# chalharu/rust-compression

Hardware: AMD Instinct MI355X
Metric: BZip2 level-9 encode MB/s (input bytes, HBM-resident in and out: the kernels' rate; value_end_to_end is host buffer to host buffer at the C ABI) (higher is better)
Workload: dtype u8/u32

## Files before the change

### rust-compression_amd/csrc/bzgpu.h

```cpp
#pragma once
#include <hip/hip_runtime.h>
#include <stdint.h>
#include <stddef.h>

namespace bzgpu {

typedef uint8_t u8;
typedef uint16_t u16;
typedef uint32_t u32;
typedef uint64_t u64;
typedef int64_t i64;

constexpr u32 kWave = 64;
constexpr u32 kMaxBlockLen = 900000;
constexpr u32 kSortTile = 8192;
constexpr u32 kSortThreads = 512;
constexpr u32 kTilesPerBlock = 110;
constexpr u32 kSlot = kTilesPerBlock * kSortTile;
constexpr u32 kPtSlot = kSlot / 8u * 10u;
constexpr u32 kPairWords = 65536u / 32u;
constexpr u32 kMaxBins = 2048;
constexpr u32 kPerK = 8;
constexpr u32 kGSize = 50;
constexpr u32 kMaxSelectors = 18002;
// ... 200 lines not shown
        if (nbytes & 1u) r = gf_mulmod(r, xp2[k]);
    return r;
}

__device__ __forceinline__ u32 crc_bytes_raw(const u8 *__restrict__ p, u64 len, const u32 *s_tab)
{
    u32 crc = 0;
    for (u64 i = 0; i < len; ++i) crc = s_tab[(crc >> 24) ^ p[i]] ^ (crc << 8);
    return crc;
}


struct RleBuffers {
    i64 *tile_last;
    i64 *carry_in;
    u32 *tile_crc;
    u32 *tile_count;
    u16 *sub_off;
    i64 *sub_rs;
    u64 *tile_off;
    u64 *total;
    u64 *cut_result;
    u64 *scan_part;
};

struct CutPlan {
    u64 L;
    u64 g_base;
    u64 own_hi;
    u64 w_min;
    u64 j_lo, j_hi;
    u64 tb, t1;
    u64 t_last;
    u64 t_eval;
};
struct CutBuffers {
    u64 *step_t0;
    u32 *step_nt;
    u64 *step_w0;
    u32 *tab;
    u16 *comp;
};

struct BwtArgs {
    const u8 *rle;
    const BlockDesc *blocks;
// ... 163 lines not shown
void launch_dec_crc(hipStream_t st, const DecArgs &a, const u64 *out_base, const u8 *out, u32 max_out_len,
                    const u32 *crc_tab, const u32 *xp2, const u32 *xp16);

enum KernelId {
    KID_RADIX_HIST = 0,
    KID_RADIX_SCAN,
    KID_RADIX_SCATTER,
    KID_GROUP_FLAGS,
    KID_GROUP_APPLY,
    KID_LAST_COLUMN,
    KID_RADIX_SCATTER_LB,
    KID_GHIST_TEXT,
    KID_GHIST_SCAN,
    KID_RANK_PLACE,
    KID_PHASE_B_LOCAL,
    KID_GROUP_REFINE,
    KID_DEC_BLOCK,
    KID_DEC_MTF,
    KID_DEC_TSORT,
    KID_DEC_WALK,
    KID_DEC_PLACE,
    KID_DEC_RLE,
    KID_DEC_CRC,
    KID_COUNT
};
struct KernelProf {
    bool on = false;
    struct Rec {
        int id;
        u64 bytes;
        hipEvent_t a, b;
    };
    Rec *recs = nullptr;
    u32 nrecs = 0, cap = 0;
    u64 launches[KID_COUNT] = {};
    u64 bytes[KID_COUNT] = {};
    double seconds[KID_COUNT] = {};
    int begin(hipStream_t st, int id, u64 nbytes);
    void end(hipStream_t st, int idx);
    void set_bytes(int idx, u64 nbytes) { if (idx >= 0) recs[idx].bytes = nbytes; }
    void collect();
    void reset();
};

void launch_slab_last(hipStream_t st, const RleBuffers &rb, u64 t0, u64 t1, i64 *d_out);
void launch_rle_scan(hipStream_t st, const u8 *d_in, u64 n, u64 t0, u64 t1, u64 in_begin, const u32 *crc_tab,
                     const u32 *xp16, const RleBuffers &rb);
void launch_rle_count(hipStream_t st, const u8 *d_in, u64 n, u64 t0, u64 t1, u64 in_begin, i64 init_carry,
                      const RleBuffers &rb, i64 *d_out_last);
void launch_rle_prefix(hipStream_t st, u64 tb, u64 t1, const RleBuffers &rb, bool write_end = true);
void launch_rle_cuts(hipStream_t st, const u8 *d_in, u64 n, u64 tb, u64 t1, u64 in_begin, const RleBuffers &rb,
                     u32 block_max_len, int emit_tail, BlockDesc *d_blocks, u32 max_blocks);
void launch_rle_image(hipStream_t st, const u8 *d_in, u64 n, u64 tb, u64 t1, u64 in_begin, const RleBuffers &rb, u8 *d_rle);
u64 cut_table_entries(const CutPlan &pl);
void cut_groups(const CutPlan &pl, u64 *g_lo, u64 *g_hi, u64 *entries);
u32 cut_seg_cap();
void launch_cut_steps(hipStream_t st, const CutPlan &pl, const RleBuffers &rb, const CutBuffers &cb);
void launch_cut_tables(hipStream_t st, const CutPlan &pl, const u8 *d_in, u64 n_lim, const RleBuffers &rb, const CutBuffers &cb,
                       u64 work_total);
void launch_cut_select(hipStream_t st, const CutPlan &pl, u64 j0, u64 s0, u64 start_in, u64 n, long long rle_bias, int emit_tail,
                       const RleBuffers &rb, const CutBuffers &cb, BlockDesc *d_blocks, u32 max_blocks);
void launch_block_crc(hipStream_t st, const u8 *d_in, const BlockDesc *d_blocks, u32 nblocks,
                      const u32 *crc_tab, const u32 *xp2, const u32 *tile_crc, u32 *d_crc);
void launch_block_symbols(hipStream_t st, const BwtArgs &a, u32 *inuse_bits, u8 *sym_code, u8 *keyinfo);
int run_bwt(hipStream_t st, const BwtArgs &a, u32 max_n, u64 total_n, unsigned long long *h_active,
            u64 *sorted_elems, KernelProf *prof, u64 *round_active , bool wide_keys,
            u32 min_chars);
void launch_mtf(hipStream_t st, const MtfArgs &a);
inline bool env_verify() { return getenv("BZ_VERIFY") && atoi(getenv("BZ_VERIFY")) != 0; }
struct MailSeg {
    void *h;
    const void *d;
    size_t n;
};
int mail_fetch(hipStream_t st, const MailSeg *segs, int nseg);
void mail_release(hipStream_t st);
// ... 12 lines not shown
```

### rust-compression_amd/csrc/engine.hip

```cpp
#include "engine_state.h"

#include <algorithm>
#include <chrono>
#include <cstdio>
#include <cstdlib>
#include <cstring>
#include <vector>

#define MAILCHK(st, ...)                                                             \
    do {                                                                             \
        const MailSeg mail_segs_[] = {__VA_ARGS__};                                  \
        if (mail_fetch((st), mail_segs_, (int)(sizeof(mail_segs_) / sizeof(mail_segs_[0]))) != 0) return BZ_E_UNEXPECTED; \
    } while (0)

static int span_begin(bz_gpu_engine *g, int stage, hipStream_t st = nullptr)
{
    bz_gpu_engine::Span s;
    s.stage = stage;
    s.st = st ? st : g->st;
    if (hipEventCreate(&s.a) != hipSuccess || hipEventCreate(&s.b) != hipSuccess) return -1;
    (void)hipEventRecord(s.a, s.st);
    g->spans.push_back(s);
    return (int)g->spans.size() - 1;
}
// ... 184 lines not shown
    df_workspace_free(g->df);
    if (g->h_active) (void)hipHostFree(g->h_active);
    mail_release(g->st);
    mail_release(g->st2);
    if (g->st) (void)hipStreamDestroy(g->st);
    if (g->ev_aux) (void)hipEventDestroy(g->ev_aux);
    if (g->st2) (void)hipStreamDestroy(g->st2);
    delete g;
}

static RleBuffers rle_buffers(bz_gpu_engine *g)
{
    RleBuffers rb;
    rb.tile_last = g->tile_last.as<i64>();
    rb.carry_in = g->carry_in.as<i64>();
    rb.tile_crc = g->tile_crc.as<u32>();
    rb.tile_count = g->tile_count.as<u32>();
    rb.tile_off = g->tile_off.as<u64>();
    rb.sub_off = g->sub_off.as<u16>();
    rb.sub_rs = g->sub_rs.as<i64>();
    rb.total = g->scal.as<u64>();
    rb.cut_result = g->scal.as<u64>() + 2;
    rb.scan_part = g->scan_part.as<u64>();
    return rb;
}

extern "C" int bz_gpu_partition_slab_begin(bz_gpu_engine *g, int level, const void *d_in, size_t n,
                                           uint64_t tile0, uint64_t tile1, int64_t *slab_last_start)
{
    if (!g || level < 1 || level > 9) return BZ_E_PARAM;
    if (n && ((uintptr_t)d_in & 15u)) return BZ_E_PARAM;
    HIPCHK(hipSetDevice(g->device));
    const u64 ntiles = (n + kRleTile - 1) / kRleTile;
    if (tile1 > ntiles) tile1 = ntiles;
    if (tile0 > tile1) tile0 = tile1;
    g->level = level;
    g->d_in = (const u8 *)d_in;
    g->n_in = n;
    g->slab_t0 = tile0;
    g->slab_t1 = tile1;
    g->h_blocks.clear();
    g->h_crc.clear();
    for (double &t : g->t_stage) t = 0;
    for (u64 &s : g->bwt_stats) s = 0;
    for (u64 &s : g->round_active) s = 0;
    if (slab_last_start) *slab_last_start = -1;
    if (ntiles == 0) return BZ_OK;
    int rc;
    if ((rc = g->tile_last.ensure(ntiles * 8)) || (rc = g->carry_in.ensure(ntiles * 8)) ||
        (rc = g->tile_crc.ensure(ntiles * 4)) || (rc = g->tile_count.ensure(ntiles * 4)) ||
        (rc = g->tile_off.ensure((ntiles + 1) * 8)) || (rc = g->sub_off.ensure(ntiles * 32)) ||
        (rc = g->sub_rs.ensure(ntiles * 128)) || (rc = g->scal.ensure(128)) ||
        (rc = g->scan_part.ensure((ntiles / 1024 + 2) * 8)))
        return rc;
    const RleBuffers rb = rle_buffers(g);
    const int sp = span_begin(g, 0);
    launch_rle_scan(g->st, g->d_in, n, tile0, tile1, 0, g->crc_tab.as<u32>(), g->xp16.as<u32>(), rb);
    i64 *d_last = reinterpret_cast<i64 *>(g->scal.as<u64>() + 8);
    if (tile1 > tile0) {
        launch_slab_last(g->st, rb, tile0, tile1, d_last);
        i64 last = -1;
        span_end(g, sp);
        MAILCHK(g->st, {&last, d_last, 8});
        if (slab_last_start) *slab_last_start = last;
    } else {
        span_end(g, sp);
    }
    HIPCHK(hipGetLastError());
    return BZ_OK;
}

extern "C" int bz_gpu_partition_slab_count(bz_gpu_engine *g, int64_t carry_run)
{
    if (!g) return BZ_E_PARAM;
    HIPCHK(hipSetDevice(g->device));
    if (g->slab_t1 <= g->slab_t0) return BZ_OK;
    const RleBuffers rb = rle_buffers(g);
    const int sp = span_begin(g, 0);
    const u64 ntiles = (g->n_in + kRleTile - 1) / kRleTile;
    launch_rle_count(g->st, g->d_in, g->n_in, g->slab_t0, g->slab_t1, 0, carry_run, rb,
                     g->slab_t1 < ntiles ? rb.carry_in + g->slab_t1 : nullptr);
    span_end(g, sp);
    HIPCHK(hipGetLastError());
    return BZ_OK;
}

struct SlabCuts {
    u64 tb = 0, start_in = 0;
    size_t nb = 0;
    int span = -1;
    bool pending = false, image_done = false;
};
static bool cut_tables_enabled()
{
    static const bool on = [] {
        const char *e = getenv("BZ_CUT_TABLES");
        return !(e && atoi(e) == 0);
    }();
    return on;
// ... 65 lines not shown
}

static int slab_cuts(bz_gpu_engine *g, uint64_t start_in, int is_last, bool image_beside, SlabCuts &sc, size_t *n_blocks,
                     uint64_t *next_in, int *tail_block)
{
    sc = SlabCuts();
    HIPCHK(hipSetDevice(g->device));
    if (n_blocks) *n_blocks = 0;
    if (next_in) *next_in = start_in;
    if (tail_block) *tail_block = 0;
    const u64 n = g->n_in;
    if (n == 0) return BZ_OK;
    const u64 t0 = g->slab_t0, t1 = g->slab_t1;
    u64 tb = start_in / kRleTile;
    if (tb > t0) tb = t0;
    if (start_in > t0 * (u64)kRleTile) return BZ_E_PARAM;
    const RleBuffers rb = rle_buffers(g);
    const u32 block_max_len = (u32)g->level * 100000u - 19u;
    sc.span = span_begin(g, 0);
    if (tb < t0) {
        launch_rle_scan(g->st, g->d_in, n, tb, t0, start_in, g->crc_tab.as<u32>(), g->xp16.as<u32>(), rb);
        launch_rle_count(g->st, g->d_in, n, tb, t0, start_in, -1, rb, nullptr);
    }
    launch_rle_prefix(g->st, tb, t1, rb);
    u64 total = 0;
    MAILCHK(g->st, {&total, rb.total, 8});
    const size_t max_blocks = (size_t)(total / block_max_len + 2);
    int rc;
    if ((rc = g->rle.ensure(total + 256)) || (rc = g->blocks_all.ensure(max_blocks * sizeof(BlockDesc))) ||
        (rc = g->crc_all.ensure(max_blocks * 4)))
        return rc;
    const bool tables = start_in == 0 && t0 == 0 && cut_tables_enabled();
    if (image_beside) {
        if (!g->ev_aux) HIPCHK(hipEventCreateWithFlags(&g->ev_aux, hipEventDisableTiming));
        if (tables) {
            launch_rle_image(g->st2, g->d_in, n, tb, t1, start_in, rb, g->rle.as<u8>());
            HIPCHK(hipEventRecord(g->ev_aux, g->st2));
            sc.image_done = true;
        }
    }
    u64 res[5] = {~0ull, 0, 0, 0, 0};
    if (tables) {
        if ((rc = cut_tables_prepare(g, 0, total, tb, t1)) != BZ_OK) return rc;
        if (g->cut_ready && (rc = cut_tables_select(g, 0, 0, 0, 0, is_last ? 1 : 0, (u32)max_blocks, res)) != BZ_OK) return rc;
        if (res[0] == ~0ull) {
            if (g->cut_ready) fprintf(stderr, "bz2_mi355x: the cut tables did not answer a target; the chain kernel takes over\n");
            ++g->cut_stats[1];
        } else {
            ++g->cut_stats[0];
        }
    }
    if (res[0] == ~0ull) {
        launch_rle_cuts(g->st, g->d_in, n, tb, t1, start_in, rb, block_max_len, is_last ? 1 : 0,
                        g->blocks_all.as<BlockDesc>(), (u32)max_blocks);
        if (image_beside && !sc.image_done) {
            launch_rle_image(g->st2, g->d_in, n, tb, t1, start_in, rb, g->rle.as<u8>());
            HIPCHK(hipEventRecord(g->ev_aux, g->st2));
            sc.image_done = true;
        }
        MAILCHK(g->st, {res, rb.cut_result, 3 * sizeof(u64)});
    }
    if (image_beside) HIPCHK(hipStreamWaitEvent(g->st, g->ev_aux, 0));
    const size_t nb = (size_t)res[0];
    if (nb > max_blocks) return BZ_E_UNEXPECTED;
    sc.tb = tb;
    sc.start_in = start_in;
    sc.nb = nb;
    sc.pending = true;
    if (n_blocks) *n_blocks = nb;
    if (next_in) *next_in = nb || is_last ? res[1] : start_in;
    if (tail_block) *tail_block = (int)res[2];
    return BZ_OK;
}
static int slab_image(bz_gpu_engine *g, SlabCuts &sc)
{
    if (!sc.pending) return BZ_OK;
    sc.pending = false;
    const RleBuffers rb = rle_buffers(g);
    if (!sc.image_done) launch_rle_image(g->st, g->d_in, g->n_in, sc.tb, g->slab_t1, sc.start_in, rb, g->rle.as<u8>());
    const size_t nb = sc.nb;
    g->h_blocks.resize(nb);
    g->h_crc.resize(nb);
    if (nb) {
        launch_block_crc(g->st, g->d_in, g->blocks_all.as<BlockDesc>(), (u32)nb, g->crc_tab.as<u32>(),
                         g->xp2.as<u32>(), g->tile_crc.as<u32>(), g->crc_all.as<u32>());
    }
    span_end(g, sc.span);
    if (nb) MAILCHK(g->st, {g->h_blocks.data(), g->blocks_all.p, nb * sizeof(BlockDesc)}, {g->h_crc.data(), g->crc_all.p, nb * 4});
    spans_collect(g);
    HIPCHK(hipGetLastError());
    return BZ_OK;
}

struct SlabSpec {
    u64 total = 0;
    u64 g_base = 0;
    u64 halo_cap = 0;
    bool image_done = false;
    u64 want_halo_total = 0;
};
static int slab_spec_total(bz_gpu_engine *g, SlabSpec &sp)
{
    sp = SlabSpec();
    if (g->n_in == 0) return BZ_OK;
    HIPCHK(hipSetDevice(g->device));
    const RleBuffers rb = rle_buffers(g);
    const int span = span_begin(g, 0);
    launch_rle_prefix(g->st, g->slab_t0, g->slab_t1, rb);
    span_end(g, span);
    MAILCHK(g->st, {&sp.total, rb.total, 8});
    return BZ_OK;
}
static int slab_spec_tables(bz_gpu_engine *g, SlabSpec &sp, u64 g_base)
{
    sp.g_base = g_base;
    g->cut_ready = false;
    if (g->n_in == 0) return BZ_OK;
    const u64 L = (u64)g->level * 100000u - 19u;
    sp.halo_cap = g_base ? (L + 8u + 255u) / 256u * 256u : 0u;
    const size_t max_blocks = (size_t)((sp.total + L + 4u) / L + 2u);
    int rc;
    if ((rc = g->rle.ensure(sp.halo_cap + sp.total + 256)) || (rc = g->blocks_all.ensure(max_blocks * sizeof(BlockDesc))) ||
        (rc = g->crc_all.ensure(max_blocks * 4)))
        return rc;
    const RleBuffers rb = rle_buffers(g);
    const int span = span_begin(g, 0);
    if (!g->ev_aux) HIPCHK(hipEventCreateWithFlags(&g->ev_aux, hipEventDisableTiming));
    launch_rle_image(g->st2, g->d_in, g->n_in, g->slab_t0, g->slab_t1, 0, rb, g->rle.as<u8>() + sp.halo_cap);
    HIPCHK(hipEventRecord(g->ev_aux, g->st2));
    sp.image_done = true;
    rc = cut_tables_prepare(g, g_base, sp.total, g->slab_t0, g->slab_t1);
    span_end(g, span);
    return rc;
}
static int slab_spec_select(bz_gpu_engine *g, SlabSpec &sp, u64 start_in, u64 s0, u64 j0, int is_last, SlabCuts &sc,
                            size_t *n_blocks, u64 *next_in, u64 *s_next, u64 *j_next)
{
    sc = SlabCuts();
    *n_blocks = 0;
    *next_in = start_in;
    *s_next = s0;
    *j_next = j0;
    if (g->n_in == 0) return BZ_OK;
    const u64 t0 = g->slab_t0;
    if (start_in > t0 * (u64)kRleTile || s0 > sp.g_base) return BZ_E_PARAM;
    const u64 L = (u64)g->level * 100000u - 19u;
    const u64 D = sp.g_base - s0;
    if (D > sp.halo_cap) return BZ_E_UNEXPECTED;
    const size_t max_blocks = (size_t)((sp.total + L + 4u) / L + 2u);
    u64 res[5] = {~0ull, 0, 0, 0, 0};
    int rc;
// ... 22 lines not shown
    sc.pending = true;
    sc.image_done = true;
    sc.span = -1;
    *n_blocks = sc.nb;
    *next_in = sc.nb || is_last ? res[1] : start_in;
    *s_next = res[3];
    *j_next = res[4];
    sp.want_halo_total = D;
    return BZ_OK;
}
static int slab_spec_finish(bz_gpu_engine *g, SlabSpec &sp, SlabCuts &sc)
{
    if (!sc.pending) return BZ_OK;
    if (!sp.image_done) return slab_image(g, sc);
    const RleBuffers rb = rle_buffers(g);
    const u64 t0 = g->slab_t0;
    sc.span = span_begin(g, 0);
    g->h_halo_total = sp.want_halo_total;
    if (sc.tb < t0) {
        launch_rle_scan(g->st, g->d_in, g->n_in, sc.tb, t0, sc.start_in, g->crc_tab.as<u32>(), g->xp16.as<u32>(), rb);
        launch_rle_count(g->st, g->d_in, g->n_in, sc.tb, t0, sc.start_in, -1, rb, nullptr);
        launch_rle_prefix(g->st, sc.tb, t0, rb, false);
        HIPCHK(hipMemcpyAsync(&g->h_halo_total, rb.total, 8, hipMemcpyDeviceToHost, g->st));
        launch_rle_image(g->st, g->d_in, g->n_in, sc.tb, t0, sc.start_in, rb, g->rle.as<u8>() + sp.halo_cap - sp.want_halo_total);
    }
    HIPCHK(hipStreamWaitEvent(g->st, g->ev_aux, 0));
    return slab_image(g, sc);
}

extern "C" int bz_gpu_partition_slab_finish(bz_gpu_engine *g, uint64_t start_in, int is_last, size_t *n_blocks,
                                            uint64_t *next_in, int *tail_block)
{
    if (!g) return BZ_E_PARAM;
    SlabCuts sc;
    const int rc = slab_cuts(g, start_in, is_last, true, sc, n_blocks, next_in, tail_block);
    if (rc != BZ_OK) {
        if (sc.span >= 0) { span_end(g, sc.span); spans_collect(g); }
        return rc;
    }
    return slab_image(g, sc);
}

extern "C" int bz_gpu_partition(bz_gpu_engine *g, int level, const void *d_in, size_t n, int mode,
                                size_t *n_blocks, size_t *consumed, int *tail_block)
{
    if (!g || level < 1 || level > 9) return BZ_E_PARAM;
    if (n_blocks) *n_blocks = 0;
// ... 931 lines not shown
        if (total >= (1u << 20)) return BZ_E_PARAM;
    }
    HIPCHK(hipSetDevice(g->device));
    DevBuf f, o, s, fl;
    int rc;
    if ((rc = f.ensure(alpha * 4)) || (rc = o.ensure(alpha + 8)) || (rc = s.ensure((size_t)kLmWords * 4)) ||
        (rc = fl.ensure(4)))
        return rc;
    HIPCHK(hipMemcpyAsync(f.p, h_freq, alpha * 4, hipMemcpyHostToDevice, g->st));
    launch_probe_code_lengths(g->st, f.as<u32>(), (u32)alpha, o.as<u8>(), s.as<u32>(), fl.as<int>());
    int flag = 0;
    HIPCHK(hipMemcpyAsync(h_len, o.p, alpha, hipMemcpyDeviceToHost, g->st));
    HIPCHK(hipMemcpyAsync(&flag, fl.p, 4, hipMemcpyDeviceToHost, g->st));
    HIPCHK(hipStreamSynchronize(g->st));
    HIPCHK(hipGetLastError());
    if (took_length_limited_path) *took_length_limited_path = flag;
    return BZ_OK;
}

static const char *kKernelNames[KID_COUNT] = {"k_radix_hist", "k_radix_scan", "k_radix_scatter",
                                              "k_group_flags", "k_group_apply", "k_last_column",
                                              "k_radix_scatter_lb", "k_ghist_text", "k_ghist_scan", "k_rank_place", "k_phase_b_local", "k_group_refine",
                                              "k_dec_block", "k_dec_mtf", "k_dec_tsort", "k_dec_walk_lengths",
                                              "k_dec_place", "k_dec_rle", "k_dec_crc"};

extern "C" int bz_gpu_profile_enable(bz_gpu_engine *g, int on)
{
    if (!g) return BZ_E_PARAM;
    g->prof.reset();
    g->prof.on = (on & 1) != 0;
    g->debug_figures = (on & 2) != 0;
    return BZ_OK;
}

extern "C" int bz_gpu_profile_kernels(bz_gpu_engine *g)
{
    (void)g;
    return KID_COUNT;
}

extern "C" int bz_gpu_profile_get(bz_gpu_engine *g, int idx, const char **name, uint64_t *launches,
                                  double *seconds, uint64_t *algorithmic_bytes)
{
    if (!g || idx < 0 || idx >= KID_COUNT) return BZ_E_PARAM;
    if (name) *name = kKernelNames[idx];
    if (launches) *launches = g->prof.launches[idx];
    if (seconds) *seconds = g->prof.seconds[idx];
// ... 4 lines not shown
```

### rust-compression_amd/csrc/engine_state.h

```cpp
#pragma once
#include "../../include/bz2_mi355x.h"
#include "bzgpu.h"
#include "dev_buf.h"

#include <cstdio>
#include <vector>

using namespace bzgpu;

struct DecWorkspace;
void dec_workspace_free(DecWorkspace *w);
int dec_decode_for_verify(struct bz_gpu_engine *g, const uint8_t *d_in, uint64_t n, uint8_t *d_out, uint64_t cap,
                          uint64_t *produced, int *verdict);
struct bz_gpu_engine *dec_cache_take(int device, int prefer = 0);
void dec_cache_put(int device, struct bz_gpu_engine *g);
void dec_release_cached();
struct DfWorkspace;
void df_workspace_free(DfWorkspace *w);

#define HIPCHK(x)                                                                                     \
    do {                                                                                              \
        hipError_t e_ = (x);                                                                          \
        if (e_ != hipSuccess) {                                                                       \
            fprintf(stderr, "bz2_mi355x: HIP error %s at %s:%d\n", hipGetErrorString(e_), __FILE__,   \
                    __LINE__);                                                                        \
            return BZ_E_UNEXPECTED;                                                                   \
        }                                                                                             \
    } while (0)

struct bz_gpu_engine {
    int device = 0;
    hipStream_t st = nullptr;
    hipStream_t st2 = nullptr;
    size_t max_blocks = 0;

    DevBuf crc_tab, xp16, xp2;
    DevBuf tile_last, carry_in, tile_crc, tile_count, tile_off, sub_off, sub_rs, scal, scan_part, rle, blocks_all, crc_all;
    DevBuf cut_step_t0, cut_step_nt, cut_step_w0, cut_tab, cut_comp;
    CutPlan cut_plan = {};
    bool cut_ready = false;
    u64 h_halo_total = 0;
    u64 cut_stats[2] = {0, 0};
    std::vector<BlockDesc> h_blocks;
    std::vector<u32> h_crc;
    const u8 *d_in = nullptr;
    u64 n_in = 0;
    u64 slab_t0 = 0, slab_t1 = 0;
    int level = 9;
    DevBuf lblocks, lcrc, SA, R, KA, VA, KB, VB, tile_hist, count, flags, tlo, tln, nonfinal, active, per_k,
        per_shift, lin_p, lin_sig, bin_cursor, pb_gate, bin_base, newbits, sym_code, keyinfo, count2, tile_nf, L, orig_ptr, inuse_bits, summ, summ_len, init_state, rank8, ptext, pair_bits, ztile_last, ztile_cnt, zstate, ztick, mtf,
        mtf_freq, bout, selector, code_len, group_bitoff, lm_scratch, hglen, hpack, hrfreq, hlm, hpass, stream, error_flag, packlist, gh_tiles, gbase,
        tile_state, tickets;
    u32 sort_epoch = 0;
    bool zle_fused_broken = false;
    u32 fused_state[2] = {0, 0};
    hipEvent_t ev_aux = nullptr;
    size_t ws_blocks = 0;
    DevBuf packed, gathered, asmlist;
    unsigned long long *h_active = nullptr;
    std::vector<BlockOut> h_out;
    std::vector<u32> h_out_nblock;
    std::vector<u32> h_out_pass;
    double t_stage[6] = {0, 0, 0, 0, 0, 0};
    KernelProf prof;
    double shard_ms[8] = {0, 0, 0, 0, 0, 0, 0, 0};
// ... 19 lines not shown
```

### rust-compression_amd/csrc/k_rle1.hip

```cpp
#include "bzgpu.h"

namespace bzgpu {

constexpr u32 RT = 256;

__device__ __forceinline__ i64 block_excl_max64(i64 v, i64 *sh , i64 &total)
{
    const u32 l = lane_id(), w = threadIdx.x >> 6;
    i64 inc = wave_incl_max64(v);
    if (l == 63) sh[w] = inc;
    __syncthreads();
    i64 carry = -1;
    for (u32 k = 0; k < w; ++k) carry = sh[k] > carry ? sh[k] : carry;
    i64 tot = -1;
    for (u32 k = 0; k < RT / 64; ++k) tot = sh[k] > tot ? sh[k] : tot;
    total = tot;
    i64 prev = __shfl_up(inc, 1, 64);
    i64 ex = (l == 0) ? (i64)-1 : prev;
    __syncthreads();
    return ex > carry ? ex : carry;
}

__device__ __forceinline__ u32 block_excl_sum(u32 v, u32 *sh , u32 &total)
{
// ... 300 lines not shown
    __shared__ __attribute__((aligned(16))) u8 s_out[2 * kRleTile + 32];
    const u64 tile = t0 + blockIdx.x;
    Seg s;
    load_seg(in, n, tile, s, in_begin);
    const i64 rs = seg_run_start(s, carry_in[tile], s_m);
    u8 e[16], cph[16];
    const u32 cnt = eval_seg(s, rs, e, cph);
    u32 tot;
    u8 *dst = rle + tile_off[tile];
    const u32 a0 = (u32)(reinterpret_cast<uintptr_t>(dst) & 15u);
    u32 o = a0 + block_excl_sum(cnt, s_s, tot);
#pragma unroll
    for (u32 k = 0; k < 16; ++k) {
        if (e[k]) {
            if (cph[k] < 4u) s_out[o++] = s.b[k];
            if (e[k] == 2u || cph[k] >= 4u) s_out[o++] = (u8)(cph[k] - 3u);
        }
    }
    __syncthreads();
    u8 *line0 = dst - a0;
    const u32 end = a0 + tot, nlines = (end + 15u) >> 4;
    for (u32 j = threadIdx.x; j < nlines; j += RT) {
        const u32 lo = j * 16u;
        if (lo >= a0 && lo + 16u <= end) {
            *reinterpret_cast<uint4 *>(line0 + lo) = *reinterpret_cast<const uint4 *>(s_out + lo);
        } else {
            const u32 b0 = lo > a0 ? lo : a0, b1 = lo + 16u < end ? lo + 16u : end;
            for (u32 b = b0; b < b1; ++b) line0[b] = s_out[b];
        }
    }
}

constexpr u32 CW = 16;
constexpr u32 CT = CW * 64;
constexpr u32 CSW_SMALL = 2, CSW_BIG = 12;
constexpr u32 CSEG = CSW_BIG * 64;
constexpr u64 CUT_END = ~0ull, CUT_OUT = ~0ull - 1;

__global__ __launch_bounds__(CT) void k_rle_cuts(const u8 *__restrict__ in, u64 n, u64 t_begin, u64 in_begin,
                                                  const u16 *__restrict__ sub_off,
                                                  const i64 *__restrict__ sub_rs,
                                                  const u64 *__restrict__ tile_off, u64 ntiles,
                                                  u32 block_max_len, int emit_tail,
                                                  BlockDesc *__restrict__ blocks, u32 max_blocks,
                                                  u64 *__restrict__ out_nblocks_consumed )
{
// ... 560 lines not shown
        if (write_end) (void)hipMemsetAsync(rb.tile_off + tb, 0, 8, st);
        return;
    }
    tiles_scan<false>(st, rb.tile_count, rb.tile_off, tb, t1, rb.scan_part, 0ull, rb.total, write_end ? rb.tile_off + t1 : nullptr);
}

void launch_rle_cuts(hipStream_t st, const u8 *d_in, u64 n, u64 tb, u64 t1, u64 in_begin, const RleBuffers &rb,
                     u32 block_max_len, int emit_tail, BlockDesc *d_blocks, u32 max_blocks)
{
    if (t1 <= tb) {
        (void)hipMemsetAsync(rb.cut_result, 0, 3 * sizeof(u64), st);
        return;
    }
    hipLaunchKernelGGL(k_rle_cuts, dim3(1), dim3(CT), 0, st, d_in, n, tb, in_begin, rb.sub_off, rb.sub_rs,
                       rb.tile_off, t1, block_max_len, emit_tail, d_blocks, max_blocks, rb.cut_result);
}
void launch_rle_image(hipStream_t st, const u8 *d_in, u64 n, u64 tb, u64 t1, u64 in_begin, const RleBuffers &rb, u8 *d_rle)
{
    if (t1 <= tb) return;
    hipLaunchKernelGGL(k_rle_scatter, dim3((u32)(t1 - tb)), dim3(RT), 0, st, d_in, n, tb, in_begin, rb.carry_in,
                       rb.tile_off, d_rle);
}

u64 cut_table_entries(const CutPlan &pl) { return pl.j_hi >= pl.j_lo ? cut_tbase(pl.j_lo, pl.j_hi + 1u) : 0u; }
void cut_groups(const CutPlan &pl, u64 *g_lo, u64 *g_hi, u64 *entries)
{
    *g_lo = (pl.j_lo + 15u) / 16u;
    *g_hi = *g_lo;
    *entries = 0;
    if (pl.j_hi < pl.j_lo || pl.j_hi + 1u < (*g_lo + 1u) * 16u) {
        *g_lo = 1;
        *g_hi = 0;
        return;
    }
    *g_hi = (pl.j_hi + 1u) / 16u - 1u;
    *entries = cut_cbase(*g_lo, *g_hi + 1u);
}
u32 cut_seg_cap() { return kCutSegCap; }
void launch_cut_steps(hipStream_t st, const CutPlan &pl, const RleBuffers &rb, const CutBuffers &cb)
{
    const u64 nsteps = pl.j_hi - pl.j_lo + 1u;
    if (nsteps == 0) return;
    hipLaunchKernelGGL(k_cut_steps, dim3((u32)((nsteps + 255u) / 256u)), dim3(256), 0, st, pl, rb.tile_off, cb.step_t0, cb.step_nt);
    tiles_scan<false>(st, cb.step_nt, cb.step_w0, 0, nsteps, cb.step_w0 + nsteps + 2, 0ull, cb.step_w0 + nsteps, nullptr);
}
void launch_cut_tables(hipStream_t st, const CutPlan &pl, const u8 *d_in, u64 n_lim, const RleBuffers &rb, const CutBuffers &cb,
// ... 32 lines not shown
```

Baseline: 14100.

## Fuse RLE1 scan, count, prefix and scatter into one decoupled look-back kernel

Adds a single-pass RLE1 front-end kernel. Each workgroup takes a span of eight tiles by atomic ticket, computes run boundaries and per-tile CRCs, and resolves the cross-span run carry and output offsets with decoupled look-back over epoch-tagged words. It then writes the RLE image directly, replacing the separate scan, slab-last, count, prefix and image kernels and one host readback on the whole-input path. The path is on by default and falls back to the three-kernel path if look-back spins time out, at the cost of extra global atomics, spin-waiting and more code complexity.

Measured after the change: 14400, median of 6. 2.1% higher.

```diff
diff --git a/rust-compression_amd/csrc/bzgpu.h b/rust-compression_amd/csrc/bzgpu.h
--- a/rust-compression_amd/csrc/bzgpu.h
+++ b/rust-compression_amd/csrc/bzgpu.h
@@ -246,6 +246,9 @@
     u64 *total;
     u64 *cut_result;
     u64 *scan_part;
+    u32 *lb_ctl;
+    u64 *lb_rs;
+    u64 *lb_off;
 };
 
 struct CutPlan {
@@ -455,6 +458,8 @@
     KID_DEC_PLACE,
     KID_DEC_RLE,
     KID_DEC_CRC,
+    KID_RLE_ONEPASS,
+    KID_RLE_SCATTER,
     KID_COUNT
 };
 struct KernelProf {
@@ -485,6 +490,10 @@
 void launch_rle_cuts(hipStream_t st, const u8 *d_in, u64 n, u64 tb, u64 t1, u64 in_begin, const RleBuffers &rb,
                      u32 block_max_len, int emit_tail, BlockDesc *d_blocks, u32 max_blocks);
 void launch_rle_image(hipStream_t st, const u8 *d_in, u64 n, u64 tb, u64 t1, u64 in_begin, const RleBuffers &rb, u8 *d_rle);
+u64 rle_onepass_spans(u64 ntiles);
+u32 rle_onepass_epochs();
+void launch_rle_onepass(hipStream_t st, const u8 *d_in, u64 n, u64 ntiles, u32 epoch, const u32 *crc_tab, const u32 *xp16,
+                        const RleBuffers &rb, u8 *d_rle, i64 *d_out_last);
 u64 cut_table_entries(const CutPlan &pl);
 void cut_groups(const CutPlan &pl, u64 *g_lo, u64 *g_hi, u64 *entries);
 u32 cut_seg_cap();
diff --git a/rust-compression_amd/csrc/engine.hip b/rust-compression_amd/csrc/engine.hip
--- a/rust-compression_amd/csrc/engine.hip
+++ b/rust-compression_amd/csrc/engine.hip
@@ -230,7 +230,62 @@
     rb.total = g->scal.as<u64>();
     rb.cut_result = g->scal.as<u64>() + 2;
     rb.scan_part = g->scan_part.as<u64>();
+    rb.lb_ctl = g->rle_lb.as<u32>();
+    rb.lb_rs = g->rle_lb.p ? reinterpret_cast<u64 *>(g->rle_lb.as<u8>() + 64) : nullptr;
+    rb.lb_off = g->rle_lb.p ? rb.lb_rs + g->rle_lb_spans : nullptr;
     return rb;
+}
+
+static bool onepass_wanted()
+{
+    static const bool on = !(getenv("BZ_RLE_ONEPASS") && atoi(getenv("BZ_RLE_ONEPASS")) == 0);
+    return on;
+}
+static bool onepass_failtest()
+{
+    static const bool on = getenv("BZ_RLE_ONEPASS_FAILTEST") && atoi(getenv("BZ_RLE_ONEPASS_FAILTEST")) != 0;
+    return on;
+}
+static void image_launch(bz_gpu_engine *g, hipStream_t st, u64 tb, u64 t1, u64 in_begin, const RleBuffers &rb, u8 *d_rle)
+{
+    if (t1 <= tb) return;
+    const int pi = g->prof.begin(st, KID_RLE_SCATTER, std::min<u64>(g->n_in, t1 * (u64)kRleTile) - tb * (u64)kRleTile);
+    launch_rle_image(st, g->d_in, g->n_in, tb, t1, in_begin, rb, d_rle);
+    g->prof.end(st, pi);
+}
+static int onepass_split(bz_gpu_engine *g, u64 ntiles, i64 *d_last, i64 *last, bool *done)
+{
+    *done = false;
+    const u64 n = g->n_in, spans = rle_onepass_spans(ntiles);
+    if (g->rle_lb.ensure(64 + spans * 16) || g->rle.ensure(n + n / 4 + 256)) {
+        (void)hipGetLastError();
+        return BZ_OK;
+    }
+    if (g->rle_lb_spans < spans || g->rle_epoch == 0 || g->rle_epoch >= rle_onepass_epochs()) {
+        g->rle_lb_spans = (g->rle_lb.cap - 64) / 16;
+        HIPCHK(hipMemsetAsync(g->rle_lb.p, 0, g->rle_lb.cap, g->st));
+        g->rle_epoch = 0;
+    }
+    ++g->rle_epoch;
+    const RleBuffers rb = rle_buffers(g);
+    const int pi = g->prof.begin(g->st, KID_RLE_ONEPASS, n);
+    launch_rle_onepass(g->st, g->d_in, n, ntiles, g->rle_epoch, g->crc_tab.as<u32>(), g->xp16.as<u32>(), rb, g->rle.as<u8>(), d_last);
+    g->prof.end(g->st, pi);
+    u32 ctl[2] = {0, 0};
+    u64 total = 0;
+    MAILCHK(g->st, {last, d_last, 8}, {&total, rb.total, 8}, {ctl, rb.lb_ctl, 8});
+    HIPCHK(hipGetLastError());
+    if (ctl[0] != (u32)spans || ctl[1] != 0 || onepass_failtest()) {
+        fprintf(stderr, "bz2_mi355x: the one-pass RLE1 front end did not complete (%u of %llu spans, error word %u); the three kernels take over\n",
+                ctl[0], (unsigned long long)spans, ctl[1]);
+        g->rle_onepass_broken = true;
+        g->rle_epoch = 0;
+        *last = -1;
+        return BZ_OK;
+    }
+    g->onepass_total = total;
+    *done = true;
+    return BZ_OK;
 }
 
 extern "C" int bz_gpu_partition_slab_begin(bz_gpu_engine *g, int level, const void *d_in, size_t n,
@@ -261,10 +316,25 @@
         (rc = g->sub_rs.ensure(ntiles * 128)) || (rc = g->scal.ensure(128)) ||
         (rc = g->scan_part.ensure((ntiles / 1024 + 2) * 8)))
         return rc;
+    const int sp = span_begin(g, 0);
+    i64 *d_last = reinterpret_cast<i64 *>(g->scal.as<u64>() + 8);
+    g->onepass_done = false;
+    if (tile0 == 0 && tile1 == ntiles && onepass_wanted() && !g->rle_onepass_broken) {
+        i64 last = -1;
+        bool done = false;
+        if ((rc = onepass_split(g, ntiles, d_last, &last, &done)) != BZ_OK) {
+            span_end(g, sp);
+            return rc;
+        }
+        if (done) {
+            g->onepass_done = true;
+            span_end(g, sp);
+            if (slab_last_start) *slab_last_start = last;
+            return BZ_OK;
+        }
+    }
     const RleBuffers rb = rle_buffers(g);
-    const int sp = span_begin(g, 0);
     launch_rle_scan(g->st, g->d_in, n, tile0, tile1, 0, g->crc_tab.as<u32>(), g->xp16.as<u32>(), rb);
-    i64 *d_last = reinterpret_cast<i64 *>(g->scal.as<u64>() + 8);
     if (tile1 > tile0) {
         launch_slab_last(g->st, rb, tile0, tile1, d_last);
         i64 last = -1;
@@ -283,6 +353,8 @@
     if (!g) return BZ_E_PARAM;
     HIPCHK(hipSetDevice(g->device));
     if (g->slab_t1 <= g->slab_t0) return BZ_OK;
+    if (g->onepass_done && carry_run == -1) return BZ_OK;
+    g->onepass_done = false;
     const RleBuffers rb = rle_buffers(g);
     const int sp = span_begin(g, 0);
     const u64 ntiles = (g->n_in + kRleTile - 1) / kRleTile;
@@ -394,19 +466,27 @@
         launch_rle_scan(g->st, g->d_in, n, tb, t0, start_in, g->crc_tab.as<u32>(), g->xp16.as<u32>(), rb);
         launch_rle_count(g->st, g->d_in, n, tb, t0, start_in, -1, rb, nullptr);
     }
-    launch_rle_prefix(g->st, tb, t1, rb);
-    u64 total = 0;
-    MAILCHK(g->st, {&total, rb.total, 8});
+    const bool onepass = g->onepass_done && start_in == 0 && t0 == 0;
+    u64 total = g->onepass_total;
+    if (!onepass) {
+        g->onepass_done = false;
+        launch_rle_prefix(g->st, tb, t1, rb);
+        MAILCHK(g->st, {&total, rb.total, 8});
+    }
     const size_t max_blocks = (size_t)(total / block_max_len + 2);
     int rc;
     if ((rc = g->rle.ensure(total + 256)) || (rc = g->blocks_all.ensure(max_blocks * sizeof(BlockDesc))) ||
         (rc = g->crc_all.ensure(max_blocks * 4)))
         return rc;
     const bool tables = start_in == 0 && t0 == 0 && cut_tables_enabled();
+    if (onepass) {
+        sc.image_done = true;
+        image_beside = false;
+    }
     if (image_beside) {
         if (!g->ev_aux) HIPCHK(hipEventCreateWithFlags(&g->ev_aux, hipEventDisableTiming));
         if (tables) {
-            launch_rle_image(g->st2, g->d_in, n, tb, t1, start_in, rb, g->rle.as<u8>());
+            image_launch(g, g->st2, tb, t1, start_in, rb, g->rle.as<u8>());
             HIPCHK(hipEventRecord(g->ev_aux, g->st2));
             sc.image_done = true;
         }
@@ -426,7 +506,7 @@
         launch_rle_cuts(g->st, g->d_in, n, tb, t1, start_in, rb, block_max_len, is_last ? 1 : 0,
                         g->blocks_all.as<BlockDesc>(), (u32)max_blocks);
         if (image_beside && !sc.image_done) {
-            launch_rle_image(g->st2, g->d_in, n, tb, t1, start_in, rb, g->rle.as<u8>());
+            image_launch(g, g->st2, tb, t1, start_in, rb, g->rle.as<u8>());
             HIPCHK(hipEventRecord(g->ev_aux, g->st2));
             sc.image_done = true;
         }
@@ -449,7 +529,7 @@
     if (!sc.pending) return BZ_OK;
     sc.pending = false;
     const RleBuffers rb = rle_buffers(g);
-    if (!sc.image_done) launch_rle_image(g->st, g->d_in, g->n_in, sc.tb, g->slab_t1, sc.start_in, rb, g->rle.as<u8>());
+    if (!sc.image_done) image_launch(g, g->st, sc.tb, g->slab_t1, sc.start_in, rb, g->rle.as<u8>());
     const size_t nb = sc.nb;
     g->h_blocks.resize(nb);
     g->h_crc.resize(nb);
@@ -476,6 +556,7 @@
     sp = SlabSpec();
     if (g->n_in == 0) return BZ_OK;
     HIPCHK(hipSetDevice(g->device));
+    g->onepass_done = false;
     const RleBuffers rb = rle_buffers(g);
     const int span = span_begin(g, 0);
     launch_rle_prefix(g->st, g->slab_t0, g->slab_t1, rb);
@@ -498,7 +579,7 @@
     const RleBuffers rb = rle_buffers(g);
     const int span = span_begin(g, 0);
     if (!g->ev_aux) HIPCHK(hipEventCreateWithFlags(&g->ev_aux, hipEventDisableTiming));
-    launch_rle_image(g->st2, g->d_in, g->n_in, g->slab_t0, g->slab_t1, 0, rb, g->rle.as<u8>() + sp.halo_cap);
+    image_launch(g, g->st2, g->slab_t0, g->slab_t1, 0, rb, g->rle.as<u8>() + sp.halo_cap);
     HIPCHK(hipEventRecord(g->ev_aux, g->st2));
     sp.image_done = true;
     rc = cut_tables_prepare(g, g_base, sp.total, g->slab_t0, g->slab_t1);
@@ -567,7 +648,7 @@
         launch_rle_count(g->st, g->d_in, g->n_in, sc.tb, t0, sc.start_in, -1, rb, nullptr);
         launch_rle_prefix(g->st, sc.tb, t0, rb, false);
         HIPCHK(hipMemcpyAsync(&g->h_halo_total, rb.total, 8, hipMemcpyDeviceToHost, g->st));
-        launch_rle_image(g->st, g->d_in, g->n_in, sc.tb, t0, sc.start_in, rb, g->rle.as<u8>() + sp.halo_cap - sp.want_halo_total);
+        image_launch(g, g->st, sc.tb, t0, sc.start_in, rb, g->rle.as<u8>() + sp.halo_cap - sp.want_halo_total);
     }
     HIPCHK(hipStreamWaitEvent(g->st, g->ev_aux, 0));
     return slab_image(g, sc);
@@ -1545,7 +1626,7 @@
                                               "k_group_flags", "k_group_apply", "k_last_column",
                                               "k_radix_scatter_lb", "k_ghist_text", "k_ghist_scan", "k_rank_place", "k_phase_b_local", "k_group_refine",
                                               "k_dec_block", "k_dec_mtf", "k_dec_tsort", "k_dec_walk_lengths",
-                                              "k_dec_place", "k_dec_rle", "k_dec_crc"};
+                                              "k_dec_place", "k_dec_rle", "k_dec_crc", "k_rle_onepass", "k_rle_scatter"};
 
 extern "C" int bz_gpu_profile_enable(bz_gpu_engine *g, int on)
 {
diff --git a/rust-compression_amd/csrc/engine_state.h b/rust-compression_amd/csrc/engine_state.h
--- a/rust-compression_amd/csrc/engine_state.h
+++ b/rust-compression_amd/csrc/engine_state.h
@@ -41,6 +41,12 @@
     bool cut_ready = false;
     u64 h_halo_total = 0;
     u64 cut_stats[2] = {0, 0};
+    DevBuf rle_lb;
+    u64 rle_lb_spans = 0;
+    u32 rle_epoch = 0;
+    bool rle_onepass_broken = false;
+    bool onepass_done = false;
+    u64 onepass_total = 0;
     std::vector<BlockDesc> h_blocks;
     std::vector<u32> h_crc;
     const u8 *d_in = nullptr;
diff --git a/rust-compression_amd/csrc/k_rle1.hip b/rust-compression_amd/csrc/k_rle1.hip
--- a/rust-compression_amd/csrc/k_rle1.hip
+++ b/rust-compression_amd/csrc/k_rle1.hip
@@ -346,6 +346,368 @@
     const u32 end = a0 + tot, nlines = (end + 15u) >> 4;
     for (u32 j = threadIdx.x; j < nlines; j += RT) {
         const u32 lo = j * 16u;
+        if (lo >= a0 && lo + 16u <= end) {
+            *reinterpret_cast<uint4 *>(line0 + lo) = *reinterpret_cast<const uint4 *>(s_out + lo);
+        } else {
+            const u32 b0 = lo > a0 ? lo : a0, b1 = lo + 16u < end ? lo + 16u : end;
+            for (u32 b = b0; b < b1; ++b) line0[b] = s_out[b];
+        }
+    }
+}
+
+constexpr u32 kSpanTiles = 8;
+constexpr u32 kSpan = kSpanTiles * kRleTile;
+constexpr u64 kOpValMask = (1ull << 46) - 1u;
+constexpr u32 kOpAgg = 1, kOpIncl = 2;
+constexpr u32 kOpEpochs = 65535;
+
+__device__ __forceinline__ u64 op_word(u32 epoch, u32 state, u64 v)
+{
+    return ((u64)epoch << 48) | ((u64)state << 46) | (v & kOpValMask);
+}
+__device__ __forceinline__ void op_publish(u64 *p, u64 w) { __hip_atomic_store(p, w, __ATOMIC_RELAXED, __HIP_MEMORY_SCOPE_AGENT); }
+
+template <bool IS_MAX> __device__ __forceinline__ bool span_look_back(const u64 *words, u64 span, u32 epoch, u32 *err, u64 &result)
+{
+    const u32 l = lane_id();
+    u64 acc = 0, hi = span;
+    u32 spins = 0;
+    while (hi > 0) {
+        const bool have = (u64)l < hi;
+        u64 w = 0;
+        if (have) w = __hip_atomic_load(words + (hi - 1u - l), __ATOMIC_RELAXED, __HIP_MEMORY_SCOPE_AGENT);
+        const u32 state = (u32)(w >> 46) & 3u;
+        const u64 val = w & kOpValMask;
+        const bool ready = have && (u32)(w >> 48) == epoch && state != 0u;
+        const bool term = ready && (state == kOpIncl || (IS_MAX && val != 0u));
+        const u64 m_wait = __ballot(have && !ready), m_term = __ballot(term);
+        const u64 m_stop = m_wait | m_term;
+        const u32 first = m_stop ? (u32)__builtin_ctzll(m_stop) : 64u;
+        if (!IS_MAX) {
+            u64 c = (have && l < first) ? val : 0u;
+#pragma unroll
+            for (u32 d = 32; d >= 1; d >>= 1) c += __shfl_xor(c, d, 64);
+            acc += c;
+        }
+        if (first < 64u && ((m_term >> first) & 1u)) {
+            const u64 tv = __shfl(val, (int)first, 64);
+            result = IS_MAX ? tv : acc + tv;
+            return true;
+        }
+        const u64 step = first < 64u ? first : 64u;
+        hi -= step < hi ? step : hi;
+        if (first < 64u) {
+            if (lb_give_up(spins, err, kLbSpinMax >> 3)) {
+                if (l == 0) __hip_atomic_store(err, 1u, __ATOMIC_RELAXED, __HIP_MEMORY_SCOPE_AGENT);
+                return false;
+            }
+            __builtin_amdgcn_s_sleep(2);
+        }
+    }
+    result = acc;
+    return true;
+}
+
+__device__ __forceinline__ u32 seg_eq_mask(const uint4 &v, int prev)
+{
+    const u32 w[4] = {v.x, v.y, v.z, v.w};
+    u32 m = 0, carry = (u32)prev & 0xFFu;
+#pragma unroll
+    for (int q = 0; q < 4; ++q) {
+        const u32 y = w[q] ^ ((w[q] << 8) | carry);
+        carry = w[q] >> 24;
+        u32 t = (y & 0x7F7F7F7Fu) + 0x7F7F7F7Fu;
+        t = ~(t | y | 0x7F7F7F7Fu);
+        const u32 u = t >> 7;
+        m |= ((u | (u >> 7) | (u >> 14) | (u >> 21)) & 0xFu) << (4 * q);
+    }
+    return prev < 0 ? m & ~1u : m;
+}
+__device__ __forceinline__ void seg_emit_masks(u32 E, u32 V, u32 c0, bool next_differs, u32 &lt4, u32 &cg)
+{
+    const u32 S = ~E & V;
+    const u32 P = (S ? (1u << __builtin_ctz(S)) - 1u : 0xFFFFu) & V;
+    const u32 wrap = 255u - c0;
+    const u32 w4 = wrap < 16u ? (0xFu << wrap) : 0u, w3 = wrap < 16u ? (0x7u << wrap) : 0u;
+    const u32 p4 = (c0 < 4u ? (1u << (4u - c0)) - 1u : 0u) | w4, p3 = (c0 < 3u ? (1u << (3u - c0)) - 1u : 0u) | w3;
+    lt4 = ((p4 & P) | S | (S << 1) | (S << 2) | (S << 3)) & V;
+    const u32 lt3 = ((p3 & P) | S | (S << 1) | (S << 2)) & V;
+    const u32 c254 = wrap >= 1u && wrap <= 16u ? (1u << (wrap - 1u)) & P : 0u;
+    const u32 top = V ^ (V >> 1);
+    const u32 ce = ((S >> 1) | (next_differs ? top : 0u) | c254) & V;
+    cg = ce & ~lt3;
+}
+
+__global__ __launch_bounds__(RT, 3) void k_rle_onepass(const u8 *__restrict__ in, u64 n, u64 ntiles, u32 nspans, u32 epoch,
+                                                     const u32 *__restrict__ crc_tab, const u32 *__restrict__ xp16,
+                                                     RleBuffers rb, u8 *__restrict__ rle, i64 *__restrict__ out_last)
+{
+    __shared__ u32 s_tab[256];
+    __shared__ int s_wmax[kSpanTiles][RT / 64];
+    __shared__ u32 s_wx[kSpanTiles][RT / 64];
+    __shared__ u32 s_wsum[kSpanTiles][RT / 64];
+    __shared__ int s_fb[kSpanTiles][RT / 64], s_lb[kSpanTiles][RT / 64];
+    __shared__ int s_edge[2];
+    __shared__ u32 s_ticket, s_fail;
+    __shared__ i64 s_carry;
+    __shared__ u32 s_cphase;
+    __shared__ u64 s_base;
+    __shared__ __attribute__((aligned(16))) u8 s_out[kSpan / 4 * 5 + 64];
+
+    const u32 tid = threadIdx.x, l = lane_id(), wv = tid >> 6;
+    if (tid == 0) {
+        s_ticket = __hip_atomic_fetch_add(rb.lb_ctl, 1u, __ATOMIC_RELAXED, __HIP_MEMORY_SCOPE_AGENT);
+        s_fail = 0;
+    }
+    s_tab[tid] = crc_tab[tid];
+    __syncthreads();
+    const u64 span = s_ticket;
+    if (span >= nspans) return;
+    const u64 B = span * (u64)kSpan;
+    u64 *w_rs = rb.lb_rs + span, *w_off = rb.lb_off + span;
+
+    uint4 v[kSpanTiles];
+    if (B + kSpan <= n) {
+#pragma unroll
+        for (u32 j = 0; j < kSpanTiles; ++j) v[j] = *reinterpret_cast<const uint4 *>(in + B + j * kRleTile + tid * 16u);
+    } else {
+#pragma unroll
+        for (u32 j = 0; j < kSpanTiles; ++j) {
+            const u64 p0 = B + j * kRleTile + tid * 16u;
+            if (p0 + 16 <= n) {
+                v[j] = *reinterpret_cast<const uint4 *>(in + p0);
+            } else {
+                u32 t[4] = {0, 0, 0, 0};
+                const u32 valid = p0 < n ? (u32)(n - p0) : 0u;
+                for (u32 k = 0; k < valid; ++k) t[k >> 2] |= (u32)in[p0 + k] << ((k & 3u) * 8u);
+                v[j] = make_uint4(t[0], t[1], t[2], t[3]);
+            }
+        }
+    }
+    if (tid == 0) {
+        s_edge[0] = B > 0 ? (int)in[B - 1] : -1;
+        s_edge[1] = B + kSpan < n ? (int)in[B + kSpan] : -1;
+    }
+#pragma unroll
+    for (u32 j = 0; j < kSpanTiles; ++j) {
+        if (l == 0) s_fb[j][wv] = (int)(v[j].x & 0xFFu);
+        if (l == 63) s_lb[j][wv] = (int)(v[j].w >> 24);
+    }
+    __syncthreads();
+    u32 pn[kSpanTiles];
+#pragma unroll
+    for (u32 j = 0; j < kSpanTiles; ++j) {
+        const u64 p0 = B + j * kRleTile + tid * 16u;
+        const u32 valid = p0 + 16 <= n ? 16u : (p0 < n ? (u32)(n - p0) : 0u);
+        int pb = __shfl_up((int)(v[j].w >> 24), 1, 64);
+        int nb = __shfl_down((int)(v[j].x & 0xFFu), 1, 64);
+        if (l == 0) pb = wv > 0 ? s_lb[j][wv - 1] : (j > 0 ? s_lb[j > 0 ? j - 1 : 0][RT / 64 - 1] : s_edge[0]);
+        if (l == 63) nb = wv + 1 < RT / 64 ? s_fb[j][wv + 1 < RT / 64 ? wv + 1 : 0] : (j + 1 < kSpanTiles ? s_fb[j + 1 < kSpanTiles ? j + 1 : 0][0] : s_edge[1]);
+        if (!(p0 > 0 && valid > 0)) pb = -1;
+        if (!(valid > 0 && p0 + valid < n)) nb = -1;
+        pn[j] = (u32)(pb + 1) | ((u32)(nb + 1) << 9);
+    }
+
+    const bool full = B + kSpan <= n;
+    u32 E[kSpanTiles];
+    int inc[kSpanTiles];
+    u32 crc[kSpanTiles];
+#pragma unroll
+    for (u32 j = 0; j < kSpanTiles; ++j) {
+        const u32 rel = j * kRleTile + tid * 16u;
+        const u32 valid = full ? 16u : (B + rel + 16 <= n ? 16u : (B + rel < n ? (u32)(n - (B + rel)) : 0u));
+        const u32 V = (1u << valid) - 1u;
+        E[j] = seg_eq_mask(v[j], (int)(pn[j] & 0x1FFu) - 1) & V;
+        const u32 S = ~E[j] & V;
+        const int last = S ? (int)(rel + 31u - (u32)__builtin_clz(S)) : -1;
+        inc[j] = wave_incl_max32(last);
+        if (l == 63) s_wmax[j][wv] = inc[j];
+        const u32 w[4] = {v[j].x, v[j].y, v[j].z, v[j].w};
+        u32 c = 0;
+#pragma unroll
+        for (u32 k = 0; k < 16; ++k)
+            if (full || k < valid) c = s_tab[(c >> 24) ^ ((w[k >> 2] >> ((k & 3u) * 8u)) & 0xFFu)] ^ (c << 8);
+        crc[j] = c;
+    }
+    if (full) {
+        u32 bx = xp16[255u - tid];
+        u32 r[kSpanTiles];
+#pragma unroll
+        for (u32 j = 0; j < kSpanTiles; ++j) r[j] = 0;
+#pragma unroll 4
+        for (u32 i = 0; i < 32; ++i) {
+#pragma unroll
+            for (u32 j = 0; j < kSpanTiles; ++j) r[j] ^= (u32)((int)(crc[j] << (31u - i)) >> 31) & bx;
+            bx = (bx << 1) ^ ((u32)((int)bx >> 31) & kCrcPoly);
+        }
+#pragma unroll
+        for (u32 j = 0; j < kSpanTiles; ++j) crc[j] = r[j];
+    } else {
+#pragma unroll
+        for (u32 j = 0; j < kSpanTiles; ++j) {
+            const u64 tile_beg = B + (u64)j * kRleTile, p0 = tile_beg + tid * 16u;
+            const u32 valid = p0 + 16 <= n ? 16u : (p0 < n ? (u32)(n - p0) : 0u);
+            if (valid > 0) {
+                const u32 tile_len = (u32)((n - tile_beg) < (u64)kRleTile ? (n - tile_beg) : (u64)kRleTile);
+                const u32 after = tile_len - (tid * 16u + valid);
+                u32 m = xp16[after >> 4];
+                for (u32 k = 0; k < (after & 15u); ++k) m = gf_mulmod(m, 0x100u);
+                crc[j] = gf_mulmod(crc[j], m);
+            } else {
+                crc[j] = 0;
+            }
+        }
+    }
+#pragma unroll
+    for (u32 j = 0; j < kSpanTiles; ++j) {
+        const u32 wx = wave_xor(crc[j]);
+        if (l == 0) s_wx[j][wv] = wx;
+    }
+    __syncthreads();
+    if (tid < kSpanTiles && span * kSpanTiles + tid < ntiles) {
+        int m = -1;
+        u32 x = 0;
+        for (u32 k = 0; k < RT / 64; ++k) {
+            m = s_wmax[tid][k] > m ? s_wmax[tid][k] : m;
+            x ^= s_wx[tid][k];
+        }
+        rb.tile_last[span * kSpanTiles + tid] = m >= 0 ? (i64)(B + (u32)m) : (i64)-1;
+        rb.tile_crc[span * kSpanTiles + tid] = x;
+    }
+    if (wv == 0) {
+        int m = l < kSpanTiles * (RT / 64) ? s_wmax[l >> 2][l & 3u] : -1;
+#pragma unroll
+        for (u32 d = 32; d >= 1; d >>= 1) {
+            const int o = __shfl_xor(m, d, 64);
+            m = o > m ? o : m;
+        }
+        const u64 own = m >= 0 ? B + (u32)m + 1u : 0u;
+        if (l == 0) op_publish(w_rs, op_word(epoch, own ? kOpIncl : kOpAgg, own));
+        u64 before = 0;
+        bool ok = true;
+        if (span > 0) ok = span_look_back<true>(rb.lb_rs, span, epoch, rb.lb_ctl + 1, before);
+        if (ok && !own && l == 0) op_publish(w_rs, op_word(epoch, kOpIncl, before));
+        if (l == 0) {
+            s_carry = (i64)before - 1;
+            s_cphase = before ? (u32)((B - (before - 1u)) % 255u) : 0u;
+            if (!ok) s_fail = 1;
+            if (ok && span + 1u == nspans && out_last) *out_last = (i64)(own ? own : before) - 1;
+        }
+    }
+    __syncthreads();
+    if (s_fail) return;
+
+    const i64 span_carry = s_carry;
+    int tcr[kSpanTiles];
+    {
+        int run = -1;
+#pragma unroll
+        for (u32 j = 0; j < kSpanTiles; ++j) {
+            tcr[j] = __builtin_amdgcn_readfirstlane(run);
+            for (u32 k = 0; k < RT / 64; ++k) run = s_wmax[j][k] > run ? s_wmax[j][k] : run;
+        }
+    }
+    const u32 cphase = s_cphase;
+    u32 exw[kSpanTiles];
+    u32 em[kSpanTiles];
+#pragma unroll
+    for (u32 j = 0; j < kSpanTiles; ++j) {
+        const int cr = tcr[j];
+        int ex = __shfl_up(inc[j], 1, 64);
+        if (l == 0) ex = -1;
+        for (u32 k = 0; k < wv; ++k) ex = s_wmax[j][k] > ex ? s_wmax[j][k] : ex;
+        if (cr > ex) ex = cr;
+        const u32 rel = j * kRleTile + tid * 16u;
+        const u32 valid = full ? 16u : (B + rel + 16 <= n ? 16u : (B + rel < n ? (u32)(n - (B + rel)) : 0u));
+        const u32 V = (1u << valid) - 1u;
+        const u32 c0 = (ex >= 0 ? rel - (u32)ex : rel + cphase) % 255u;
+        pn[j] |= c0 << 18;
+        const int nxt = (int)((pn[j] >> 9) & 0x1FFu) - 1;
+        u32 lastb = v[j].w >> 24;
+        if (valid != 16u && valid > 0u) {
+            const u32 w[4] = {v[j].x, v[j].y, v[j].z, v[j].w};
+            lastb = 0;
+#pragma unroll
+            for (u32 k = 0; k < 16; ++k)
+                if (k + 1u == valid) lastb = (w[k >> 2] >> ((k & 3u) * 8u)) & 0xFFu;
+        }
+        u32 lt4, cg;
+        seg_emit_masks(E[j], V, c0, nxt != (int)lastb, lt4, cg);
+        em[j] = lt4 | (cg << 16);
+        const u32 cnt = (u32)__builtin_popcount(em[j]);
+        const u32 incs = wave_incl_sum(cnt);
+        exw[j] = incs - cnt;
+        if (l == 63) s_wsum[j][wv] = incs;
+        const u64 tile = span * kSpanTiles + j;
+        if (tile < ntiles) {
+            if (tid == 0) rb.carry_in[tile] = cr >= 0 ? (i64)(B + (u32)cr) : span_carry;
+            if ((tid & 15u) == 0) rb.sub_rs[tile * 16u + (tid >> 4)] = ex >= 0 ? (i64)(B + (u32)ex) : span_carry;
+        }
+    }
+    __syncthreads();
+    u32 tile_ex[kSpanTiles];
+    u32 span_total = 0;
+#pragma unroll
+    for (u32 j = 0; j < kSpanTiles; ++j) {
+        tile_ex[j] = span_total;
+        u32 below = 0, tot = 0;
+        for (u32 k = 0; k < RT / 64; ++k) {
+            if (k < wv) below += s_wsum[j][k];
+            tot += s_wsum[j][k];
+        }
+        exw[j] += (u32)__builtin_amdgcn_readfirstlane((int)below);
+        span_total += (u32)__builtin_amdgcn_readfirstlane((int)tot);
+        const u64 tile = span * kSpanTiles + j;
+        if (tile < ntiles) {
+            if (tid == 0) rb.tile_count[tile] = tot;
+            if ((tid & 15u) == 0) rb.sub_off[tile * 16u + (tid >> 4)] = (u16)exw[j];
+        }
+    }
+    if (wv == 0) {
+        if (l == 0) op_publish(w_off, op_word(epoch, span ? kOpAgg : kOpIncl, span_total));
+        u64 base = 0;
+        bool ok = true;
+        if (span > 0) {
+            ok = span_look_back<false>(rb.lb_off, span, epoch, rb.lb_ctl + 1, base);
+            if (ok && l == 0) op_publish(w_off, op_word(epoch, kOpIncl, base + span_total));
+        }
+        if (l == 0) {
+            s_base = base;
+            if (!ok) s_fail = 1;
+            if (ok && span + 1u == nspans) {
+                rb.tile_off[ntiles] = base + span_total;
+                *rb.total = base + span_total;
+            }
+        }
+    }
+    __syncthreads();
+    if (s_fail) return;
+    const u64 base = s_base;
+#pragma unroll
+    for (u32 j = 0; j < kSpanTiles; ++j)
+        if (tid == j && span * kSpanTiles + j < ntiles) rb.tile_off[span * kSpanTiles + j] = base + tile_ex[j];
+
+    u8 *dst = rle + base;
+    const u32 a0 = (u32)(reinterpret_cast<uintptr_t>(dst) & 15u);
+#pragma unroll
+    for (u32 j = 0; j < kSpanTiles; ++j) {
+        const u32 w[4] = {v[j].x, v[j].y, v[j].z, v[j].w};
+        const u32 lt4 = em[j] & 0xFFFFu, cg = em[j] >> 16, S = ~E[j];
+        u32 o = a0 + tile_ex[j] + exw[j];
+        u32 c = pn[j] >> 18;
+#pragma unroll
+        for (u32 k = 0; k < 16; ++k) {
+            if ((S >> k) & 1u) c = 0;
+            if ((lt4 >> k) & 1u) s_out[o++] = (u8)(w[k >> 2] >> ((k & 3u) * 8u));
+            if ((cg >> k) & 1u) s_out[o++] = (u8)(c - 3u);
+            c = c == 254u ? 0u : c + 1u;
+        }
+    }
+    __syncthreads();
+    u8 *line0 = dst - a0;
+    const u32 end = a0 + span_total, nlines = (end + 15u) >> 4;
+    for (u32 q = tid; q < nlines; q += RT) {
+        const u32 lo = q * 16u;
         if (lo >= a0 && lo + 16u <= end) {
             *reinterpret_cast<uint4 *>(line0 + lo) = *reinterpret_cast<const uint4 *>(s_out + lo);
         } else {
@@ -952,6 +1314,16 @@
                        rb.tile_off, d_rle);
 }
 
+u64 rle_onepass_spans(u64 ntiles) { return (ntiles + kSpanTiles - 1u) / kSpanTiles; }
+u32 rle_onepass_epochs() { return kOpEpochs; }
+void launch_rle_onepass(hipStream_t st, const u8 *d_in, u64 n, u64 ntiles, u32 epoch, const u32 *crc_tab, const u32 *xp16,
+                        const RleBuffers &rb, u8 *d_rle, i64 *d_out_last)
+{
+    (void)hipMemsetAsync(rb.lb_ctl, 0, 16, st);
+    hipLaunchKernelGGL(k_rle_onepass, dim3((u32)rle_onepass_spans(ntiles)), dim3(RT), 0, st, d_in, n, ntiles,
+                       (u32)rle_onepass_spans(ntiles), epoch, crc_tab, xp16, rb, d_rle, d_out_last);
+}
+
 u64 cut_table_entries(const CutPlan &pl) { return pl.j_hi >= pl.j_lo ? cut_tbase(pl.j_lo, pl.j_hi + 1u) : 0u; }
 void cut_groups(const CutPlan &pl, u64 *g_lo, u64 *g_hi, u64 *entries)
 {
```
